# crockwell/rel_pose

Measured on AMD Instinct MI355X. Metric: image-pairs/sec fwd+bwd @384x384, 1/2/4/8 MI355X; R,t err vs ref, higher is better.
Workload: dtype f32; 1 GPU; train.py step (ViTEss fwd + geodesic loss + bwd + grad all-reduce + clip + Adam), synthetic 384x384 pairs; scope=full, pairs_per_gpu=64, global_batch_pairs=64, parallelism=dp1, finite=True, gemm_operand_precision=exact fp32 MFMA, launch=eager

## Files before the change

### rel_pose_amd/csrc/attention.hip

```cpp
#include "common.h"
#include "../../include/relpose_hip.h"
#include <stdlib.h>
#include <type_traits>

namespace {

template <int OFF> RP_DEV float lds_rd32(unsigned addr) {
  float v;
  asm volatile("ds_read_b32 %0, %1 offset:%2" : "=v"(v) : "v"(addr), "n"(OFF));
  return v;
}
template <int N, class F> RP_DEV void static_for(F&& f) {
  if constexpr (N > 0) {
    static_for<N - 1>(f);
    f(std::integral_constant<int, N - 1>{});
  }
}

constexpr int NTOK = 576;
constexpr int KST = 68;
constexpr int NTILE = NTOK / 32;

struct AttnP {
  const float* q; const float* k; const float* v;
  float* o; float* lse;
  int H, ldq, ldk, ldv, ldo, q_xor, k_xor;
  float scale;
  int ZH;
  float* colpart;
  float* pst;
  float* mrun;
};

template <int NT>
RP_DEV void tile_gload(const float* base, int ld, int tid, float4 (&r)[(512 + NT - 1) / NT]) {
#pragma unroll
  for (int j = 0; j < (512 + NT - 1) / NT; ++j) {
    int f = tid + NT * j;
    if (512 % NT != 0) f = min(f, 511);
    r[j] = ld4(base + (long long)(f >> 4) * ld + (f & 15) * 4);
  }
}
template <int NT, int STRIDE>
RP_DEV void tile_sstore(float* s, int tid, const float4 (&r)[(512 + NT - 1) / NT]) {
#pragma unroll
  for (int j = 0; j < (512 + NT - 1) / NT; ++j) {
    int f = tid + NT * j;
    if (512 % NT != 0) f = min(f, 511);
    st4(s + (f >> 4) * STRIDE + (f & 15) * 4, r[j]);
  }
}

template <bool BF>
RP_DEV f32x16 score_tile(const float* Ks, int l31, int hi, const float (&breg)[32], const bf16x8 (&bpk)[4]) {
  f32x16 s = zero16();
  const float* kr = Ks + l31 * KST + 32 * hi;
  if (BF) {
#pragma unroll
    for (int c = 0; c < 4; ++c) {
      const float4 x = ld4(kr + 8 * c), y = ld4(kr + 8 * c + 4);
      s = mfma_bf(pack8(x.x, x.y, x.z, x.w, y.x, y.y, y.z, y.w), bpk[c], s);
    }
    return s;
  }
#pragma unroll
  for (int c = 0; c < 8; ++c) {
    const float4 kf = ld4(kr + 4 * c);
    s = mfma32(kf.x, breg[4 * c + 0], s);
    s = mfma32(kf.y, breg[4 * c + 1], s);
    s = mfma32(kf.z, breg[4 * c + 2], s);
    s = mfma32(kf.w, breg[4 * c + 3], s);
  }
  return s;
}

template <int STRIDE, bool BF>
RP_DEV void accum_tile(const float* Ts, int l31, int hi, const f32x16& p, f32x16& o0, f32x16& o1) {
  if (BF) {
#pragma unroll
    for (int g = 0; g < 2; ++g) {
      float a0[8], a1[8];
#pragma unroll
      for (int j = 0; j < 8; ++j) {
        const float* vr = Ts + acc_row(8 * g + j, hi) * STRIDE + l31;
        a0[j] = vr[0];
        a1[j] = vr[32];
      }
      const bf16x8 pb = pack8(p[8 * g], p[8 * g + 1], p[8 * g + 2], p[8 * g + 3], p[8 * g + 4], p[8 * g + 5], p[8 * g + 6], p[8 * g + 7]);
      o0 = mfma_bf(pack8(a0), pb, o0);
      o1 = mfma_bf(pack8(a1), pb, o1);
    }
    return;
  }
#pragma unroll
  for (int r = 0; r < 16; ++r) {
    const float* vr = Ts + acc_row(r, hi) * STRIDE + l31;
    o0 = mfma32(vr[0], p[r], o0);
    o1 = mfma32(vr[32], p[r], o1);
  }
}

RP_DEV void store_ownerT(float* row_ptr, int hi, const f32x16& o0, const f32x16& o1, float mul) {
#pragma unroll
  for (int g = 0; g < 4; ++g) {
    st4(row_ptr + 8 * g + 4 * hi, make_float4(o0[4 * g] * mul, o0[4 * g + 1] * mul, o0[4 * g + 2] * mul, o0[4 * g + 3] * mul));
    st4(row_ptr + 32 + 8 * g + 4 * hi, make_float4(o1[4 * g] * mul, o1[4 * g + 1] * mul, o1[4 * g + 2] * mul, o1[4 * g + 3] * mul));
  }
}

RP_DEV void colsum_ownerT(float* part, int l31, int hi, const f32x16& o0, const f32x16& o1, float mul) {
#pragma unroll
  for (int r = 0; r < 16; ++r) {
    float a = row16_sum(o0[r]), b = row16_sum(o1[r]);
    a += __shfl_xor(a, 16, 64);
    b += __shfl_xor(b, 16, 64);
    if (l31 == 0) {
      part[acc_row(r, hi)] = a * mul;
      part[32 + acc_row(r, hi)] = b * mul;
    }
  }
}

RP_DEV void load_owner(const float* row_ptr, int hi, float mul, float (&reg)[32]) {
#pragma unroll
  for (int c = 0; c < 8; ++c) {
    const float4 x = ld4(row_ptr + 32 * hi + 4 * c);
    reg[4 * c + 0] = x.x * mul; reg[4 * c + 1] = x.y * mul; reg[4 * c + 2] = x.z * mul; reg[4 * c + 3] = x.w * mul;
  }
}

RP_DEV void pack_owner(const float (&reg)[32], bf16x8 (&pk)[4]) {
#pragma unroll
  for (int c = 0; c < 4; ++c) pk[c] = pack8(&reg[8 * c]);
}

template <bool NTS = true>
RP_DEV void store_tile_runs(float* tile, const f32x16& v, int lane) {
  typedef float f4v __attribute__((ext_vector_type(4)));
#pragma unroll
  for (int g = 0; g < 4; ++g) {
    const f4v x = {v[4 * g], v[4 * g + 1], v[4 * g + 2], v[4 * g + 3]};
    if (NTS) __builtin_nontemporal_store(x, reinterpret_cast<f4v*>(tile + 4 * (64 * g + lane)));
    else *reinterpret_cast<f4v*>(tile + 4 * (64 * g + lane)) = x;
  }
}

template <int NW, bool STATS, int WPS, bool BF, bool COLS = false, bool SAVEP = false>
__global__ __launch_bounds__(NW * 64, WPS) void attn_fwd_kernel(AttnP p) {
  constexpr int NT = NW * 64;
  constexpr int NPF = (512 + NT - 1) / NT;
  __shared__ __attribute__((aligned(16))) float Ks[2][32 * KST];
  __shared__ __attribute__((aligned(16))) float Vs[STATS ? 1 : 2][STATS ? 4 : 32 * 64];
  const int tid = threadIdx.x, lane = tid & 63, wave = tid >> 6, l31 = lane & 31, hi = lane >> 5;
  int zh, qblk;
  if (!xcd_problem(NTILE / NW, p.ZH, zh, qblk)) return;
  const int h = zh % p.H, z = zh / p.H;
  const int q0 = (qblk * NW + wave) * 32;
  const float* qb = p.q + (long long)(z ^ p.q_xor) * NTOK * p.ldq + h * 64;
  const float* kb = p.k + (long long)(z ^ (p.k_xor & 1)) * NTOK * p.ldk + h * 64;
  const float* vb = STATS ? nullptr : p.v + (long long)(z ^ (p.k_xor >> 1)) * NTOK * p.ldv + h * 64;

  float qreg[32];
  load_owner(qb + (long long)(q0 + l31) * p.ldq, hi, p.scale * RP_LOG2E, qreg);
  bf16x8 qpk[4];
  if (BF) pack_owner(qreg, qpk);

  f32x16 o0 = zero16(), o1 = zero16();
  float m = -INFINITY, l = 0.f;

  float4 kpre[NPF], vpre[NPF];
  tile_gload<NT>(kb, p.ldk, tid, kpre);
  if (!STATS) tile_gload<NT>(vb, p.ldv, tid, vpre);
  tile_sstore<NT, KST>(Ks[0], tid, kpre);
  if (!STATS) tile_sstore<NT, 64>(Vs[0], tid, vpre);
  __syncthreads();

  const int krow = l31 * KST + 32 * hi;
  float4 ka[4], kb2[4];
#pragma unroll
  for (int c = 0; c < 4; ++c) ka[c] = ld4(Ks[0] + krow + 4 * c);

  tile_gload<NT>(kb + (long long)32 * p.ldk, p.ldk, tid, kpre);
  if (!STATS) tile_gload<NT>(vb + (long long)32 * p.ldv, p.ldv, tid, vpre);

  for (int t = 0; t < NTILE; ++t) {
    const int cur = t & 1;
    const bool more = t + 1 < NTILE;
    float va[16], vb_[16];
#pragma unroll
    for (int c = 0; c < 4; ++c) kb2[c] = ld4(Ks[cur] + krow + 16 + 4 * c);
    if (!STATS) {
#pragma unroll
      for (int r = 0; r < 8; ++r) {
        const float* vr = Vs[cur] + acc_row(r, hi) * 64 + l31;
        va[2 * r] = vr[0];
        va[2 * r + 1] = vr[32];
      }
    }
    __builtin_amdgcn_sched_barrier(0);
    f32x16 s = zero16();
    if (BF) {
      s = mfma_bf(pack8(ka[0].x, ka[0].y, ka[0].z, ka[0].w, ka[1].x, ka[1].y, ka[1].z, ka[1].w), qpk[0], s);
      s = mfma_bf(pack8(ka[2].x, ka[2].y, ka[2].z, ka[2].w, ka[3].x, ka[3].y, ka[3].z, ka[3].w), qpk[1], s);
      s = mfma_bf(pack8(kb2[0].x, kb2[0].y, kb2[0].z, kb2[0].w, kb2[1].x, kb2[1].y, kb2[1].z, kb2[1].w), qpk[2], s);
      s = mfma_bf(pack8(kb2[2].x, kb2[2].y, kb2[2].z, kb2[2].w, kb2[3].x, kb2[3].y, kb2[3].z, kb2[3].w), qpk[3], s);
    } else {
#pragma unroll
    for (int c = 0; c < 4; ++c) {
      s = mfma32(ka[c].x, qreg[4 * c + 0], s);
      s = mfma32(ka[c].y, qreg[4 * c + 1], s);
      s = mfma32(ka[c].z, qreg[4 * c + 2], s);
      s = mfma32(ka[c].w, qreg[4 * c + 3], s);
    }
#pragma unroll
    for (int c = 0; c < 4; ++c) {
      s = mfma32(kb2[c].x, qreg[16 + 4 * c + 0], s);
      s = mfma32(kb2[c].y, qreg[16 + 4 * c + 1], s);
      s = mfma32(kb2[c].z, qreg[16 + 4 * c + 2], s);
      s = mfma32(kb2[c].w, qreg[16 + 4 * c + 3], s);
    }
    }
    if (STATS && SAVEP)
      store_tile_runs<false>(p.pst + (((long long)zh * NTILE + (q0 >> 5)) * NTILE + t) * 1024, s, lane);
    if (COLS) {
      float2* cp = reinterpret_cast<float2*>(p.colpart) + ((long long)zh * NTILE + (q0 >> 5)) * NTOK + t * 32;
#pragma unroll
      for (int r = 0; r < 16; ++r) {
        float cm = row16_max(s[r]);
        cm = fmaxf(cm, __shfl_xor(cm, 16, 64));
        float cl = row16_sum(fast_exp2(s[r] - cm));
        cl += __shfl_xor(cl, 16, 64);
        cp[acc_row(r, hi)] = make_float2(cm, cl);
      }
    }
    float mx = s[0];
#pragma unroll
    for (int r = 1; r < 16; ++r) mx = fmaxf(mx, s[r]);
    mx = fmaxf(mx, __shfl_xor(mx, 32, 64));
    const float mn = fmaxf(m, mx);
    const float alpha = fast_exp2(m - mn);
    m = mn;
    float ps = 0.f;
#pragma unroll
    for (int r = 0; r < 16; ++r) {
      s[r] = fast_exp2(s[r] - mn);
      ps += s[r];
    }
    l = l * alpha + ps;
    if (SAVEP && !STATS) {
      store_tile_runs(p.pst + (((long long)zh * NTILE + (q0 >> 5)) * NTILE + t) * 1024, s, lane);
      p.mrun[((long long)zh * NTILE + t) * NTOK + q0 + l31] = mn;
    }
    if (!STATS) {
#pragma unroll
      for (int r = 0; r < 8; ++r) {
        const float* vr = Vs[cur] + acc_row(8 + r, hi) * 64 + l31;
        vb_[2 * r] = vr[0];
        vb_[2 * r + 1] = vr[32];
      }
#pragma unroll
      for (int r = 0; r < 16; ++r) {
        o0[r] *= alpha;
        o1[r] *= alpha;
      }
      __builtin_amdgcn_sched_barrier(0);
      if (BF) {
        const bf16x8 pb = pack8(s[0], s[1], s[2], s[3], s[4], s[5], s[6], s[7]);
        o0 = mfma_bf(pack8(va[0], va[2], va[4], va[6], va[8], va[10], va[12], va[14]), pb, o0);
        o1 = mfma_bf(pack8(va[1], va[3], va[5], va[7], va[9], va[11], va[13], va[15]), pb, o1);
      } else {
#pragma unroll
      for (int r = 0; r < 8; ++r) {
        o0 = mfma32(va[2 * r], s[r], o0);
        o1 = mfma32(va[2 * r + 1], s[r], o1);
      }
      }
    }
    if (more) {
      tile_sstore<NT, KST>(Ks[cur ^ 1], tid, kpre);
      if (!STATS) tile_sstore<NT, 64>(Vs[cur ^ 1], tid, vpre);
    }
    __syncthreads();
    if (more) {
#pragma unroll
      for (int c = 0; c < 4; ++c) ka[c] = ld4(Ks[cur ^ 1] + krow + 4 * c);
      if (t + 2 < NTILE) {
        tile_gload<NT>(kb + (long long)(t + 2) * 32 * p.ldk, p.ldk, tid, kpre);
        if (!STATS) tile_gload<NT>(vb + (long long)(t + 2) * 32 * p.ldv, p.ldv, tid, vpre);
      }
    }
    if (!STATS) {
      __builtin_amdgcn_sched_barrier(0);
      if (BF) {
        const bf16x8 pb = pack8(s[8], s[9], s[10], s[11], s[12], s[13], s[14], s[15]);
        o0 = mfma_bf(pack8(vb_[0], vb_[2], vb_[4], vb_[6], vb_[8], vb_[10], vb_[12], vb_[14]), pb, o0);
        o1 = mfma_bf(pack8(vb_[1], vb_[3], vb_[5], vb_[7], vb_[9], vb_[11], vb_[13], vb_[15]), pb, o1);
      } else {
#pragma unroll
      for (int r = 0; r < 8; ++r) {
        o0 = mfma32(vb_[2 * r], s[8 + r], o0);
        o1 = mfma32(vb_[2 * r + 1], s[8 + r], o1);
      }
      }
    }
  }
  const float lt = l + __shfl_xor(l, 32, 64);
  if (!STATS) store_ownerT(p.o + ((long long)z * NTOK + q0 + l31) * p.ldo + h * 64, hi, o0, o1, 1.0f / lt);
  if (hi == 0) p.lse[((long long)z * p.H + h) * NTOK + q0 + l31] = m * RP_LN2 + logf(lt);
}

struct AttnBwdP {
  const float* q; const float* k; const float* v; const float* dout; const float* lse; const float* delta;
  float* dq; float* dk; float* dv;
  int H, ldq, ldk, ldv, lddo, lddq, lddk, lddv;
  float scale;
  int ZH;
  int kv_xor;
  float* ds;
  float *dk_colpart, *dv_colpart;
  int ldp;
  const float* pst;
  const float* mrun;
};

#ifdef RP_DKDV_PROBE
__device__ unsigned long long g_probe[16];
#define STAMP(i) { const unsigned long long now_ = __builtin_readcyclecounter(); acc_[i] += now_ - last_; last_ = now_; }
#else
#define STAMP(i)
#endif
template <int NW, int WPS, bool BF>
__global__ __launch_bounds__(NW * 64, WPS) void attn_bwd_dkdv_kernel(AttnBwdP p) {
#ifdef RP_DKDV_PROBE
  unsigned long long acc_[8] = {0, 0, 0, 0, 0, 0, 0, 0}, last_ = __builtin_readcyclecounter();
#endif
  constexpr int NT = NW * 64;
  constexpr int NPF = (512 + NT - 1) / NT;
  __shared__ __attribute__((aligned(16))) float Qs[2][32 * KST];
  __shared__ __attribute__((aligned(16))) float Ds[2][32 * KST];
  __shared__ __attribute__((aligned(16))) float Ls[2][64];
  __shared__ __attribute__((aligned(16))) float Tst[BF ? 1 : NW][BF ? 4 : 512];
  const int tid = threadIdx.x, lane = tid & 63, wave = tid >> 6, l31 = lane & 31, hi = lane >> 5;
  int zh, qblk;
  if (!xcd_problem(NTILE / NW, p.ZH, zh, qblk)) return;
  const int h = zh % p.H, z = zh / p.H;
  const int k0 = (qblk * NW + wave) * 32;
  const int zq = z ^ p.kv_xor;
  const float* qb = p.q + (long long)zq * NTOK * p.ldq + h * 64;
  const float* dob = p.dout + (long long)zq * NTOK * p.lddo + h * 64;
  const float* lseb = p.lse + ((long long)zq * p.H + h) * NTOK;
  const float* delb = p.delta + ((long long)zq * p.H + h) * NTOK;

  float kreg[32], vreg[32];
  load_owner(p.k + ((long long)z * NTOK + k0 + l31) * p.ldk + h * 64, hi, p.scale * RP_LOG2E, kreg);
  load_owner(p.v + ((long long)z * NTOK + k0 + l31) * p.ldv + h * 64, hi, 1.0f, vreg);
  bf16x8 kpk[4], vpk[4];
  if (BF) { pack_owner(kreg, kpk); pack_owner(vreg, vpk); }

  f32x16 dv0 = zero16(), dv1 = zero16(), dk0 = zero16(), dk1 = zero16();
  float4 qpre[NPF], dpre[NPF];
  float lpre = 0.f;
  tile_gload<NT>(qb, p.ldq, tid, qpre);
  tile_gload<NT>(dob, p.lddo, tid, dpre);
  const float* lsrc = (lane & 32) ? delb + (lane & 31) : lseb + (lane & 31);
  const float lmul = (lane & 32) ? 1.0f : RP_LOG2E;
  lpre = lsrc[0] * lmul;
  tile_sstore<NT, KST>(Qs[0], tid, qpre);
  tile_sstore<NT, KST>(Ds[0], tid, dpre);
  if (tid < 64) Ls[0][tid] = lpre;
  __syncthreads();

  STAMP(0)
  for (int t = 0; t < NTILE; ++t) {
    const int cur = t & 1;
    if (t + 1 < NTILE) {
      tile_gload<NT>(qb + (long long)(t + 1) * 32 * p.ldq, p.ldq, tid, qpre);
      tile_gload<NT>(dob + (long long)(t + 1) * 32 * p.lddo, p.lddo, tid, dpre);
      lpre = lsrc[(t + 1) * 32] * lmul;
    }
    STAMP(1)
    f32x16 s = score_tile<BF>(Qs[cur], l31, hi, kreg, kpk);
    f32x16 dp = score_tile<BF>(Ds[cur], l31, hi, vreg, vpk);
#ifdef RP_DKDV_PROBE
    asm volatile("" : "+v"(s), "+v"(dp));
#endif
    STAMP(2)
#pragma unroll
    for (int r = 0; r < 16; ++r) {
      const int qi = acc_row(r, hi);
      const float pr = fast_exp2(s[r] - Ls[cur][qi]);
      s[r] = pr;
      dp[r] = pr * (dp[r] - Ls[cur][32 + qi]);
    }
#ifdef RP_DKDV_PROBE
    asm volatile("" : "+v"(s), "+v"(dp));
#endif
    STAMP(3)
    if (p.ds) {
      const long long tile = (((long long)zq * p.H + h) * NTILE + t) * NTILE + (k0 >> 5);
      if (BF) store_acc_image_bf16(reinterpret_cast<unsigned short*>(p.ds) + tile * 1024, dp, p.scale, lane);
      else store_acc_image_lds(p.ds + tile * 1024, Tst[BF ? 0 : wave], dp, p.scale, lane);
    }
    STAMP(4)
    accum_tile<KST, BF>(Ds[cur], l31, hi, s, dv0, dv1);
    accum_tile<KST, BF>(Qs[cur], l31, hi, dp, dk0, dk1);
#ifdef RP_DKDV_PROBE
    asm volatile("" : "+v"(dv0), "+v"(dv1), "+v"(dk0), "+v"(dk1));
#endif
    STAMP(5)
    if (t + 1 < NTILE) {
      tile_sstore<NT, KST>(Qs[cur ^ 1], tid, qpre);
      tile_sstore<NT, KST>(Ds[cur ^ 1], tid, dpre);
      if (tid < 64) Ls[cur ^ 1][tid] = lpre;
    }
    STAMP(6)
    __syncthreads();
    STAMP(7)
  }
#ifdef RP_DKDV_PROBE
  if (lane == 0) { for (int i = 0; i < 8; ++i) atomicAdd(&g_probe[i], acc_[i]); atomicAdd(&g_probe[8], 1ull); }
#endif
  store_ownerT(p.dv + ((long long)z * NTOK + k0 + l31) * p.lddv + h * 64, hi, dv0, dv1, 1.0f);
  store_ownerT(p.dk + ((long long)z * NTOK + k0 + l31) * p.lddk + h * 64, hi, dk0, dk1, p.scale);
  if (p.dk_colpart) {
    const long long prow = ((long long)z * NTILE + (k0 >> 5)) * p.ldp + h * 64;
    colsum_ownerT(p.dv_colpart + prow, l31, hi, dv0, dv1, 1.0f);
    colsum_ownerT(p.dk_colpart + prow, l31, hi, dk0, dk1, p.scale);
  }
}

template <int NW, int WPS>
__global__ __launch_bounds__(NW * 64, WPS) void attn_bwd_dkdv_p_kernel(AttnBwdP p) {
#ifdef RP_DKDV_PROBE
  unsigned long long acc_[8] = {0, 0, 0, 0, 0, 0, 0, 0}, last_ = __builtin_readcyclecounter();
#endif
  constexpr int NT = NW * 64;
  constexpr int NPF = (512 + NT - 1) / NT;
  __shared__ __attribute__((aligned(16))) float Qs[2][32 * KST];
  __shared__ __attribute__((aligned(16))) float Ds[2][32 * KST];
  __shared__ __attribute__((aligned(16))) float Ls[2][NW][64];
  const int tid = threadIdx.x, lane = tid & 63, wave = tid >> 6, l31 = lane & 31, hi = lane >> 5;
  int zh, qblk;
  if (!xcd_problem(NTILE / NW, p.ZH, zh, qblk)) return;
  const int h = zh % p.H, z = zh / p.H;
  const int kb = qblk * NW + wave, k0 = kb * 32;
  const float* qb = p.q + (long long)z * NTOK * p.ldq + h * 64;
  const float* dob = p.dout + (long long)z * NTOK * p.lddo + h * 64;
  const float* lseb = p.lse + (long long)zh * NTOK;
  const float* delb = p.delta + (long long)zh * NTOK;
  const float* mb = p.mrun + ((long long)zh * NTILE + kb) * NTOK;
  const float* pt = p.pst + ((long long)zh * NTILE * NTILE + kb) * 1024 + (l31 >> 2) * 128 + (l31 & 3) + 16 * hi;
  float* dst = p.ds + ((long long)zh * NTILE * NTILE + kb) * 1024;

  float vreg[32];
  load_owner(p.v + ((long long)z * NTOK + k0 + l31) * p.ldv + h * 64, hi, p.scale, vreg);
  const bf16x8 nopk[4] = {};
  f32x16 dv0 = zero16(), dv1 = zero16(), dk0 = zero16(), dk1 = zero16();
  float4 qpre[NPF], dpre[NPF];
  const float* asrc = (lane & 32) ? delb + l31 : lseb + l31;
  const float* bsrc = (lane & 32) ? delb + l31 : mb + l31;
  const float km = (lane & 32) ? p.scale : 0.f, ke = (lane & 32) ? 0.f : 1.f;
  auto lfac = [&](float a, float b) { return fmaf(km, a, ke * fast_exp2(ke * fmaf(-a, RP_LOG2E, b))); };
  auto pload = [&](f32x16& x, int t) {
    const float* tp = pt + (long long)t * (NTILE * 1024);
#pragma unroll
    for (int r = 0; r < 16; ++r) x[r] = tp[acc_row(r, 0) * 4];
  };
  f32x16 pa, pb;
  tile_gload<NT>(qb, p.ldq, tid, qpre);
  tile_gload<NT>(dob, p.lddo, tid, dpre);
  float la = asrc[0], lb = bsrc[0];
  pload(pa, 0);
  tile_sstore<NT, KST>(Qs[0], tid, qpre);
  tile_sstore<NT, KST>(Ds[0], tid, dpre);
  Ls[0][wave][lane] = lfac(la, lb);
  __syncthreads();

  auto step = [&](f32x16& pc, f32x16& pn, int t) {
    const int cur = t & 1;
    if (t + 1 < NTILE) {
      tile_gload<NT>(qb + (long long)(t + 1) * 32 * p.ldq, p.ldq, tid, qpre);
      tile_gload<NT>(dob + (long long)(t + 1) * 32 * p.lddo, p.lddo, tid, dpre);
      la = asrc[(t + 1) * 32];
      lb = bsrc[(t + 1) * 32];
      pload(pn, t + 1);
    }
    STAMP(1)
    f32x16 dp = score_tile<false>(Ds[cur], l31, hi, vreg, nopk);
#ifdef RP_DKDV_PROBE
    asm volatile("" : "+v"(dp));
#endif
    STAMP(2)
    const float* L = Ls[cur][wave];
#pragma unroll
    for (int r = 0; r < 16; ++r) {
      const int qi = acc_row(r, hi);
      pc[r] *= L[qi];
      dp[r] = pc[r] * (dp[r] - L[32 + qi]);
    }
#ifdef RP_DKDV_PROBE
    asm volatile("" : "+v"(dp), "+v"(pc));
#endif
    STAMP(3)
    store_tile_runs(dst + (long long)t * (NTILE * 1024), dp, lane);
    STAMP(4)
    accum_tile<KST, false>(Ds[cur], l31, hi, pc, dv0, dv1);
    accum_tile<KST, false>(Qs[cur], l31, hi, dp, dk0, dk1);
#ifdef RP_DKDV_PROBE
    asm volatile("" : "+v"(dv0), "+v"(dv1), "+v"(dk0), "+v"(dk1));
#endif
    STAMP(5)
    if (t + 1 < NTILE) {
      tile_sstore<NT, KST>(Qs[cur ^ 1], tid, qpre);
      tile_sstore<NT, KST>(Ds[cur ^ 1], tid, dpre);
      Ls[cur ^ 1][wave][lane] = lfac(la, lb);
    }
    STAMP(6)
    __syncthreads();
    STAMP(7)
  };
  for (int t = 0; t < NTILE; t += 2) {
    step(pa, pb, t);
    step(pb, pa, t + 1);
  }
#ifdef RP_DKDV_PROBE
  if (lane == 0) { for (int i = 0; i < 8; ++i) atomicAdd(&g_probe[i], acc_[i]); atomicAdd(&g_probe[8], 1ull); }
#endif
  store_ownerT(p.dv + ((long long)z * NTOK + k0 + l31) * p.lddv + h * 64, hi, dv0, dv1, 1.0f);
  store_ownerT(p.dk + ((long long)z * NTOK + k0 + l31) * p.lddk + h * 64, hi, dk0, dk1, 1.0f);
  if (p.dk_colpart) {
    const long long prow = ((long long)z * NTILE + kb) * p.ldp + h * 64;
    colsum_ownerT(p.dv_colpart + prow, l31, hi, dv0, dv1, 1.0f);
    colsum_ownerT(p.dk_colpart + prow, l31, hi, dk0, dk1, 1.0f);
  }
}

template <int NW, int WPS, bool BF>
__global__ __launch_bounds__(NW * 64, WPS) void attn_bwd_dq_kernel(AttnBwdP p) {
  constexpr int NT = NW * 64;
  constexpr int NPF = (512 + NT - 1) / NT;
  __shared__ __attribute__((aligned(16))) float Ks[2][32 * KST];
  __shared__ __attribute__((aligned(16))) float Vs[2][32 * KST];
  const int tid = threadIdx.x, lane = tid & 63, wave = tid >> 6, l31 = lane & 31, hi = lane >> 5;
  int zh, qblk;
  if (!xcd_problem(NTILE / NW, p.ZH, zh, qblk)) return;
  const int h = zh % p.H, z = zh / p.H;
  const int q0 = (qblk * NW + wave) * 32;
  const float* kb = p.k + (long long)(z ^ p.kv_xor) * NTOK * p.ldk + h * 64;
  const float* vb = p.v + (long long)(z ^ p.kv_xor) * NTOK * p.ldv + h * 64;

  float qreg[32], dreg[32];
  load_owner(p.q + ((long long)z * NTOK + q0 + l31) * p.ldq + h * 64, hi, p.scale * RP_LOG2E, qreg);
  load_owner(p.dout + ((long long)z * NTOK + q0 + l31) * p.lddo + h * 64, hi, 1.0f, dreg);
  bf16x8 qpk[4], dpk[4];
  if (BF) { pack_owner(qreg, qpk); pack_owner(dreg, dpk); }
  const float lse = p.lse[((long long)z * p.H + h) * NTOK + q0 + l31] * RP_LOG2E;
  const float del = p.delta[((long long)z * p.H + h) * NTOK + q0 + l31];

  f32x16 dq0 = zero16(), dq1 = zero16();
  float4 kpre[NPF], vpre[NPF];
  tile_gload<NT>(kb, p.ldk, tid, kpre);
  tile_gload<NT>(vb, p.ldv, tid, vpre);
  tile_sstore<NT, KST>(Ks[0], tid, kpre);
  tile_sstore<NT, KST>(Vs[0], tid, vpre);
  __syncthreads();
  for (int t = 0; t < NTILE; ++t) {
    const int cur = t & 1;
    if (t + 1 < NTILE) {
      tile_gload<NT>(kb + (long long)(t + 1) * 32 * p.ldk, p.ldk, tid, kpre);
      tile_gload<NT>(vb + (long long)(t + 1) * 32 * p.ldv, p.ldv, tid, vpre);
    }
    f32x16 s = score_tile<BF>(Ks[cur], l31, hi, qreg, qpk);
    f32x16 dp = score_tile<BF>(Vs[cur], l31, hi, dreg, dpk);
#pragma unroll
    for (int r = 0; r < 16; ++r) dp[r] = fast_exp2(s[r] - lse) * (dp[r] - del);
    accum_tile<KST, BF>(Ks[cur], l31, hi, dp, dq0, dq1);
    if (t + 1 < NTILE) {
      tile_sstore<NT, KST>(Ks[cur ^ 1], tid, kpre);
      tile_sstore<NT, KST>(Vs[cur ^ 1], tid, vpre);
    }
    __syncthreads();
  }
  store_ownerT(p.dq + ((long long)z * NTOK + q0 + l31) * p.lddq + h * 64, hi, dq0, dq1, p.scale);
}

struct DsMmP {
  const float* ds; const float* b; float* out;
  int H, ldb, ldo, b_xor, ZH;
  int reverse;
  float* colpart;
  int ldp;
};

RP_DEV void accum_rows16(const float* Ts, int l31, int hi, const f32x16& p, f32x16& o0, f32x16& o1) {
#pragma unroll
  for (int r = 0; r < 16; ++r) {
    const float* vr = Ts + (16 * hi + r) * 64 + l31;
    o0 = mfma32(vr[0], p[r], o0);
    o1 = mfma32(vr[32], p[r], o1);
  }
}

template <int NW>
__global__ __launch_bounds__(NW * 64, 4) void ds_matmul_kernel(DsMmP p) {
  constexpr int NT = NW * 64;
  constexpr int KT = 32;
  constexpr int NSTEP = NTOK / KT;
  constexpr int NPF = (KT * 16 + NT - 1) / NT;
  __shared__ __attribute__((aligned(16))) float Bs[2][KT * 64];
  const int tid = threadIdx.x, lane = tid & 63, wave = tid >> 6, l31 = lane & 31, hi = lane >> 5;
  int zh, blk;
  if (!xcd_problem(NTILE / NW, p.ZH, zh, blk)) return;
  if (p.reverse) zh = p.ZH - 1 - zh;
  const int h = zh % p.H, z = zh / p.H;
  const int i0 = (blk * NW + wave) * 32;
  const float* bb = p.b + (long long)(z ^ p.b_xor) * NTOK * p.ldb + h * 64;
  const float* arow = p.ds + ((long long)zh * NTILE + (i0 >> 5)) * NTILE * 1024 + ((l31 & 3) + 4 * (l31 >> 3)) * 64 + 32 * ((l31 >> 2) & 1) + 16 * hi;

  f32x16 o0 = zero16(), o1 = zero16();
  float4 bpre[NPF];
  constexpr int NA = KT / 8;
  float4 a0[NA], a1[NA], a2[NA];
  auto aload = [&](float4 (&a)[NA], int t) {
#pragma unroll
    for (int g = 0; g < NA; ++g) {
      const float* src = arow + 1024 * ((KT / 32) * t + (g >> 2)) + 4 * (g & 3);
      a[g] = ld4(src);
    }
  };
  auto bload = [&](int t) {
#pragma unroll
    for (int j = 0; j < NPF; ++j) {
      int f = tid + NT * j;
      if ((KT * 16) % NT != 0) f = min(f, KT * 16 - 1);
      bpre[j] = ld4(bb + (long long)(t * KT + (f >> 4)) * p.ldb + (f & 15) * 4);
    }
  };
  auto bstore = [&](float* dst) {
#pragma unroll
    for (int j = 0; j < NPF; ++j) {
      int f = tid + NT * j;
      if ((KT * 16) % NT != 0) f = min(f, KT * 16 - 1);
      st4(dst + f * 4, bpre[j]);
    }
  };
  bload(0);
  aload(a0, 0);
  aload(a1, 1);
  bstore(Bs[0]);
  __syncthreads();
  bload(1);
  auto step = [&](const float4 (&a)[NA], float4 (&anext)[NA], int t) {
    const int cur = t & 1;
    if (t + 2 < NSTEP) aload(anext, t + 2);
#pragma unroll
    for (int u = 0; u < KT / 32; ++u) {
      f32x16 pr;
#pragma unroll
      for (int g = 0; g < 4; ++g) { pr[4 * g] = a[4 * u + g].x; pr[4 * g + 1] = a[4 * u + g].y; pr[4 * g + 2] = a[4 * u + g].z; pr[4 * g + 3] = a[4 * u + g].w; }
      accum_rows16(Bs[cur] + u * 32 * 64, l31, hi, pr, o0, o1);
    }
    if (t + 1 < NSTEP) bstore(Bs[cur ^ 1]);
    __syncthreads();
    if (t + 2 < NSTEP) bload(t + 2);
  };
  for (int t = 0; t < NSTEP; t += 3) {
    step(a0, a2, t);
    step(a1, a0, t + 1);
    step(a2, a1, t + 2);
  }
  store_ownerT(p.out + ((long long)z * NTOK + i0 + l31) * p.ldo + h * 64, hi, o0, o1, 1.0f);
  if (p.colpart) colsum_ownerT(p.colpart + ((long long)z * NTILE + (i0 >> 5)) * p.ldp + h * 64, l31, hi, o0, o1, 1.0f);
}

template <int NW>
__global__ __launch_bounds__(NW * 64, 3) void ds_matmul_t_kernel(DsMmP p) {
  __shared__ __attribute__((aligned(16))) float Bs[2][32 * 64];
  __shared__ __attribute__((aligned(16))) float Dt[NW][2][1024];
  const int tid = threadIdx.x, lane = tid & 63, wave = __builtin_amdgcn_readfirstlane(tid >> 6), l31 = lane & 31, hi = lane >> 5;
  int zh, blk;
  if (!xcd_problem(NTILE / NW, p.ZH, zh, blk)) return;
  if (p.reverse) zh = p.ZH - 1 - zh;
  const int h = zh % p.H, z = zh / p.H;
  const int ib = blk * NW + wave, i0 = ib * 32;
  const float* bb = p.b + (long long)(z ^ p.b_xor) * NTOK * p.ldb + h * 64;
  const float* tiles = p.ds + ((long long)zh * NTILE + ib) * NTILE * 1024;
  constexpr int BP = (8 + NW - 1) / NW;
  const unsigned dvoff = ((lane & 7) * 32 + (lane >> 3)) * 16, bvoff = (unsigned)((lane >> 4) * p.ldb * 4 + (lane & 15) * 16);
  const unsigned dt0 = lds_byte_addr(&Dt[wave][0][0]), bs0 = lds_byte_addr(&Bs[0][0]);
  auto issue = [&](int t, int buf) {
    const float* ts = tiles + (long long)t * 1024;
#pragma unroll
    for (int c = 0; c < 4; ++c) glds16(uniform_ptr(ts + 32 * c), dvoff, dt0 + buf * 4096 + c * 1024);
#pragma unroll
    for (int c = 0; c < BP; ++c) {
      const int piece = min(wave + NW * c, 7);
      glds16(uniform_ptr(bb + (long long)(t * 32 + 4 * piece) * p.ldb), bvoff, bs0 + buf * 8192 + piece * 1024);
    }
  };
  f32x16 o0 = zero16(), o1 = zero16();
  issue(0, 0);
  asm volatile("s_waitcnt vmcnt(0)" ::: "memory");
  __syncthreads();
  for (int t = 0; t < NTILE; ++t) {
    const int cur = t & 1;
    if (t + 1 < NTILE) issue(t + 1, cur ^ 1);
    const float* B = Bs[cur] + hi * 64 + l31;
    const float* D = Dt[wave][cur] + hi * 32 + l31;
#pragma unroll
    for (int s = 0; s < 16; ++s) {
      const float dsv = D[64 * s];
      o0 = mfma32(B[128 * s], dsv, o0);
      o1 = mfma32(B[128 * s + 32], dsv, o1);
    }
    asm volatile("s_waitcnt vmcnt(0)" ::: "memory");
    __syncthreads();
  }
  store_ownerT(p.out + ((long long)z * NTOK + i0 + l31) * p.ldo + h * 64, hi, o0, o1, 1.0f);
  if (p.colpart) colsum_ownerT(p.colpart + ((long long)z * NTILE + ib) * p.ldp + h * 64, l31, hi, o0, o1, 1.0f);
}

template <int NW>
__global__ __launch_bounds__(NW * 64, 3) void ds_matmul_t16_kernel(DsMmP p) {
  __shared__ __attribute__((aligned(16))) float Bs[2][32 * 64];
  __shared__ __attribute__((aligned(16))) float Dt[NW][2][1024];
  const int tid = threadIdx.x, lane = tid & 63, wave = __builtin_amdgcn_readfirstlane(tid >> 6), l15 = lane & 15, kq = lane >> 4;
  int zh, blk;
  if (!xcd_problem(NTILE / NW, p.ZH, zh, blk)) return;
  if (p.reverse) zh = p.ZH - 1 - zh;
  const int h = zh % p.H, z = zh / p.H;
  const int ib = blk * NW + wave, i0 = ib * 32;
  const float* bb = p.b + (long long)(z ^ p.b_xor) * NTOK * p.ldb + h * 64;
  const float* tiles = p.ds + ((long long)zh * NTILE + ib) * NTILE * 1024;
  constexpr int BP = (8 + NW - 1) / NW;
  const unsigned dvoff = ((((lane & 7) ^ (4 * ((lane >> 4) & 1))) * 32) + (lane >> 3)) * 16;
  const unsigned bvoff = (unsigned)((lane >> 4) * p.ldb * 4 + (((lane & 15) ^ (4 * (lane >> 4))) * 16));
  const unsigned dt0 = lds_byte_addr(&Dt[wave][0][0]), bs0 = lds_byte_addr(&Bs[0][0]);
  auto issue = [&](int t, int buf) {
    const float* ts = tiles + (long long)t * 1024;
#pragma unroll
    for (int c = 0; c < 4; ++c) glds16(uniform_ptr(ts + 32 * c), dvoff, dt0 + buf * 4096 + c * 1024);
#pragma unroll
    for (int c = 0; c < BP; ++c) {
      const int piece = min(wave + NW * c, 7);
      glds16(uniform_ptr(bb + (long long)(t * 32 + 4 * piece) * p.ldb), bvoff, bs0 + buf * 8192 + piece * 1024);
    }
  };
  f32x4 acc[4][2];
#pragma unroll
  for (int m = 0; m < 4; ++m)
#pragma unroll
    for (int n = 0; n < 2; ++n) acc[m][n] = f32x4{0.f, 0.f, 0.f, 0.f};
  int aoff[4], boff[2];
#pragma unroll
  for (int m = 0; m < 4; ++m) aoff[m] = kq * 64 + 16 * (m ^ kq) + l15;
#pragma unroll
  for (int n = 0; n < 2; ++n) boff[n] = kq * 32 + 16 * (n ^ (kq >> 1)) + l15;
  issue(0, 0);
  asm volatile("s_waitcnt vmcnt(0)" ::: "memory");
  __syncthreads();
  for (int t = 0; t < NTILE; ++t) {
    const int cur = t & 1;
    if (t + 1 < NTILE) issue(t + 1, cur ^ 1);
    const float* B = Bs[cur];
    const float* D = Dt[wave][cur];
#pragma unroll
    for (int ks = 0; ks < 8; ++ks) {
      float av[4], bv[2];
#pragma unroll
      for (int m = 0; m < 4; ++m) av[m] = B[ks * 256 + aoff[m]];
#pragma unroll
      for (int n = 0; n < 2; ++n) bv[n] = D[ks * 128 + boff[n]];
#pragma unroll
      for (int m = 0; m < 4; ++m)
#pragma unroll
        for (int n = 0; n < 2; ++n) acc[m][n] = __builtin_amdgcn_mfma_f32_16x16x4f32(av[m], bv[n], acc[m][n], 0, 0, 0);
    }
    asm volatile("s_waitcnt vmcnt(0)" ::: "memory");
    __syncthreads();
  }
#pragma unroll
  for (int n = 0; n < 2; ++n) {
    float* orow = p.out + ((long long)z * NTOK + i0 + 16 * n + l15) * p.ldo + h * 64 + 4 * kq;
#pragma unroll
    for (int m = 0; m < 4; ++m) st4(orow + 16 * m, make_float4(acc[m][n][0], acc[m][n][1], acc[m][n][2], acc[m][n][3]));
  }
  if (p.colpart) {
    float* part = p.colpart + ((long long)z * NTILE + ib) * p.ldp + h * 64;
#pragma unroll
    for (int m = 0; m < 4; ++m)
#pragma unroll
      for (int e = 0; e < 4; ++e) {
        const float v = row16_sum(acc[m][0][e] + acc[m][1][e]);
        if (l15 == 0) part[16 * m + 4 * kq + e] = v;
      }
  }
}

template <int NW>
__global__ __launch_bounds__(NW * 64, 4) void ds_matmul_bf16_kernel(DsMmP p) {
  constexpr int NT = NW * 64;
  constexpr int NPF = (512 + NT - 1) / NT;
  __shared__ __attribute__((aligned(16))) float Bs[2][32 * 64];
  const int tid = threadIdx.x, lane = tid & 63, wave = tid >> 6, l31 = lane & 31, hi = lane >> 5;
  int zh, blk;
  if (!xcd_problem(NTILE / NW, p.ZH, zh, blk)) return;
  if (p.reverse) zh = p.ZH - 1 - zh;
  const int h = zh % p.H, z = zh / p.H;
  const int i0 = (blk * NW + wave) * 32;
  const float* bb = p.b + (long long)(z ^ p.b_xor) * NTOK * p.ldb + h * 64;
  const unsigned short* arow = reinterpret_cast<const unsigned short*>(p.ds) + ((long long)zh * NTILE + (i0 >> 5)) * NTILE * 1024 +
                               ((l31 & 3) + 4 * (l31 >> 3)) * 64 + 32 * ((l31 >> 2) & 1) + 16 * hi;
  f32x16 o0 = zero16(), o1 = zero16();
  float4 bpre[NPF];
  uint4 a0[2], a1[2], a2[2];
  auto aload = [&](uint4 (&a)[2], int t) {
    a[0] = *reinterpret_cast<const uint4*>(arow + 1024 * t);
    a[1] = *reinterpret_cast<const uint4*>(arow + 1024 * t + 8);
  };
  auto bload = [&](int t) {
#pragma unroll
    for (int j = 0; j < NPF; ++j) {
      int f = tid + NT * j;
      if (512 % NT != 0) f = min(f, 511);
      bpre[j] = ld4(bb + (long long)(t * 32 + (f >> 4)) * p.ldb + (f & 15) * 4);
    }
// ... 321 lines not shown
```

Baseline: 1998 image-pairs/sec.

## Stream Q/dO tiles into swizzled LDS via direct global-to-LDS loads in dK/dV kernel

Reworks the attention backward dK/dV (P-stored) kernel so the Q and dO tiles go straight from global memory into XOR-swizzled LDS buffers through direct global-to-LDS loads. This replaces the old path of loading into registers and then storing to padded shared memory. New swizzle-aware score and accumulate helpers read those buffers, and the next tile's loads are issued between the two accumulate phases. Global accesses use address_space(1) pointers with uniform bases, and the wave index is made scalar. The aim is to cut register pressure and VALU/LDS store traffic and to overlap loads with MFMA work. The cost is hand-placed waitcnt and scheduling code that is fragile to get right.

```diff
diff --git a/rel_pose_amd/csrc/attention.hip b/rel_pose_amd/csrc/attention.hip
--- a/rel_pose_amd/csrc/attention.hip
+++ b/rel_pose_amd/csrc/attention.hip
@@ -134,14 +134,18 @@
   for (int c = 0; c < 4; ++c) pk[c] = pack8(&reg[8 * c]);
 }
 
-template <bool NTS = true>
-RP_DEV void store_tile_runs(float* tile, const f32x16& v, int lane) {
+template <bool NTS = true, class TP = float*, class LT = int>
+RP_DEV void store_tile_runs(TP tile, const f32x16& v, LT lane) {
   typedef float f4v __attribute__((ext_vector_type(4)));
+  typedef decltype(reinterpret_cast<f4v*>((float*)nullptr)) generic_t;
+  typedef __attribute__((address_space(1))) f4v* global_t;
+  typedef std::conditional_t<std::is_same<TP, float*>::value, generic_t, global_t> vp_t;
+  const TP mine = tile + 4 * lane;
 #pragma unroll
   for (int g = 0; g < 4; ++g) {
     const f4v x = {v[4 * g], v[4 * g + 1], v[4 * g + 2], v[4 * g + 3]};
-    if (NTS) __builtin_nontemporal_store(x, reinterpret_cast<f4v*>(tile + 4 * (64 * g + lane)));
-    else *reinterpret_cast<f4v*>(tile + 4 * (64 * g + lane)) = x;
+    if (NTS) __builtin_nontemporal_store(x, (vp_t)(mine + 256 * g));
+    else *(vp_t)(mine + 256 * g) = x;
   }
 }
 
@@ -429,17 +433,41 @@
   }
 }
 
+typedef const __attribute__((address_space(1))) float* rp_gcptr_t;
+typedef __attribute__((address_space(1))) float* rp_gptr_t;
+RP_DEV rp_gcptr_t uniform_gptr(const float* p) { return (rp_gcptr_t)(unsigned long long)uniform_ptr(p); }
+RP_DEV f32x16 score_tile_sw(const float* T, const int (&sc)[8], const float (&breg)[32]) {
+  f32x16 s = zero16();
+#pragma unroll
+  for (int c = 0; c < 8; ++c) {
+    const float4 kf = ld4(T + sc[c]);
+    s = mfma32(kf.x, breg[4 * c + 0], s);
+    s = mfma32(kf.y, breg[4 * c + 1], s);
+    s = mfma32(kf.z, breg[4 * c + 2], s);
+    s = mfma32(kf.w, breg[4 * c + 3], s);
+  }
+  return s;
+}
+template <bool VOL>
+RP_DEV void accum_tile_sw(const float* T, const int (&ar)[4], const f32x16& p, f32x16& o0, f32x16& o1) {
+#pragma unroll
+  for (int r = 0; r < 16; ++r) {
+    typedef std::conditional_t<VOL, const volatile __attribute__((address_space(3))) float*, const float*> rd_t;
+    const rd_t vr = (rd_t)T + ar[r & 3] + (r >> 2) * 512;
+    const int b = (r >> 2) & 1;
+    o0 = mfma32(vr[32 * b], p[r], o0);
+    o1 = mfma32(vr[32 * (1 - b)], p[r], o1);
+  }
+}
+
 template <int NW, int WPS>
 __global__ __launch_bounds__(NW * 64, WPS) void attn_bwd_dkdv_p_kernel(AttnBwdP p) {
 #ifdef RP_DKDV_PROBE
   unsigned long long acc_[8] = {0, 0, 0, 0, 0, 0, 0, 0}, last_ = __builtin_readcyclecounter();
 #endif
-  constexpr int NT = NW * 64;
-  constexpr int NPF = (512 + NT - 1) / NT;
-  __shared__ __attribute__((aligned(16))) float Qs[2][32 * KST];
-  __shared__ __attribute__((aligned(16))) float Ds[2][32 * KST];
+  __shared__ __attribute__((aligned(16))) float Ts[2][2][32 * 64];
   __shared__ __attribute__((aligned(16))) float Ls[2][NW][64];
-  const int tid = threadIdx.x, lane = tid & 63, wave = tid >> 6, l31 = lane & 31, hi = lane >> 5;
+  const int tid = threadIdx.x, lane = tid & 63, wave = __builtin_amdgcn_readfirstlane(tid >> 6), l31 = lane & 31, hi = lane >> 5;
   int zh, qblk;
   if (!xcd_problem(NTILE / NW, p.ZH, zh, qblk)) return;
   const int h = zh % p.H, z = zh / p.H;
@@ -449,44 +477,65 @@
   const float* lseb = p.lse + (long long)zh * NTOK;
   const float* delb = p.delta + (long long)zh * NTOK;
   const float* mb = p.mrun + ((long long)zh * NTILE + kb) * NTOK;
-  const float* pt = p.pst + ((long long)zh * NTILE * NTILE + kb) * 1024 + (l31 >> 2) * 128 + (l31 & 3) + 16 * hi;
+  const float* ptile = p.pst + ((long long)zh * NTILE * NTILE + kb) * 1024;
+  const unsigned poff = (l31 >> 2) * 128 + (l31 & 3) + 16 * hi;
   float* dst = p.ds + ((long long)zh * NTILE * NTILE + kb) * 1024;
 
   float vreg[32];
   load_owner(p.v + ((long long)z * NTOK + k0 + l31) * p.ldv + h * 64, hi, p.scale, vreg);
-  const bf16x8 nopk[4] = {};
   f32x16 dv0 = zero16(), dv1 = zero16(), dk0 = zero16(), dk1 = zero16();
-  float4 qpre[NPF], dpre[NPF];
-  const float* asrc = (lane & 32) ? delb + l31 : lseb + l31;
-  const float* bsrc = (lane & 32) ? delb + l31 : mb + l31;
+  constexpr int NV = 4 / NW, NI = 8 / NW;
+  unsigned qvoff[NV], dvoff[NV];
+#pragma unroll
+  for (int j = 0; j < NV; ++j) {
+    const unsigned x = (((lane & 15) ^ (lane >> 4) ^ (4 * (j * NW + wave))) & 15) * 16;
+    qvoff[j] = (unsigned)((lane >> 4) * p.ldq * 4) + x;
+    dvoff[j] = (unsigned)((lane >> 4) * p.lddo * 4) + x;
+  }
+  const unsigned ts0 = lds_byte_addr(&Ts[0][0][0]) + wave * 1024;
+  const long long qstep = (long long)(4 * NW) * p.ldq, dstep = (long long)(4 * NW) * p.lddo;
+  auto issue = [&](int t, int buf) {
+    const float* qs = uniform_ptr(qb + (long long)(t * 32 + 4 * wave) * p.ldq);
+    const float* dd = uniform_ptr(dob + (long long)(t * 32 + 4 * wave) * p.lddo);
+#pragma unroll
+    for (int i = 0; i < NI; ++i) glds16(qs + i * qstep, qvoff[i % NV], ts0 + buf * 16384 + i * (NW * 1024));
+#pragma unroll
+    for (int i = 0; i < NI; ++i) glds16(dd + i * dstep, dvoff[i % NV], ts0 + buf * 16384 + 8192 + i * (NW * 1024));
+  };
+  int sc[8], ar[4];
+#pragma unroll
+  for (int c = 0; c < 8; ++c) sc[c] = l31 * 64 + (((8 * hi + c) ^ (l31 & 15)) << 2);
+#pragma unroll
+  for (int j = 0; j < 4; ++j) ar[j] = (j + 4 * hi) * 64 + ((((l31 >> 2) ^ (j + 4 * hi)) << 2) | (l31 & 3));
   const float km = (lane & 32) ? p.scale : 0.f, ke = (lane & 32) ? 0.f : 1.f;
-  auto lfac = [&](float a, float b) { return fmaf(km, a, ke * fast_exp2(ke * fmaf(-a, RP_LOG2E, b))); };
+  auto lfac = [&](float lse, float del, float m) { return fmaf(km, del, ke * fast_exp2(ke * fmaf(-lse, RP_LOG2E, m))); };
+  float la, ld, lm;
+  auto lload = [&](int t) {
+    la = (uniform_gptr(lseb + t * 32) + (unsigned)l31)[0];
+    ld = (uniform_gptr(delb + t * 32) + (unsigned)l31)[0];
+    lm = (uniform_gptr(mb + t * 32) + (unsigned)l31)[0];
+  };
   auto pload = [&](f32x16& x, int t) {
-    const float* tp = pt + (long long)t * (NTILE * 1024);
+    const rp_gcptr_t tp = uniform_gptr(ptile + (long long)t * (NTILE * 1024)) + poff;
 #pragma unroll
     for (int r = 0; r < 16; ++r) x[r] = tp[acc_row(r, 0) * 4];
   };
   f32x16 pa, pb;
-  tile_gload<NT>(qb, p.ldq, tid, qpre);
-  tile_gload<NT>(dob, p.lddo, tid, dpre);
-  float la = asrc[0], lb = bsrc[0];
+  issue(0, 0);
+  lload(0);
   pload(pa, 0);
-  tile_sstore<NT, KST>(Qs[0], tid, qpre);
-  tile_sstore<NT, KST>(Ds[0], tid, dpre);
-  Ls[0][wave][lane] = lfac(la, lb);
+  asm volatile("s_waitcnt vmcnt(0)" ::: "memory");
+  Ls[0][wave][lane] = lfac(la, ld, lm);
   __syncthreads();
 
-  auto step = [&](f32x16& pc, f32x16& pn, int t) {
-    const int cur = t & 1;
-    if (t + 1 < NTILE) {
-      tile_gload<NT>(qb + (long long)(t + 1) * 32 * p.ldq, p.ldq, tid, qpre);
-      tile_gload<NT>(dob + (long long)(t + 1) * 32 * p.lddo, p.lddo, tid, dpre);
-      la = asrc[(t + 1) * 32];
-      lb = bsrc[(t + 1) * 32];
-      pload(pn, t + 1);
-    }
+  auto step = [&](f32x16& pc, f32x16& pn, int t, auto curc) {
+    constexpr int cur = decltype(curc)::value;
+    const int tn = cur ? min(t + 1, NTILE - 1) : t + 1;
+    lload(tn);
+    pload(pn, tn);
+    asm volatile("" ::: "memory");
     STAMP(1)
-    f32x16 dp = score_tile<false>(Ds[cur], l31, hi, vreg, nopk);
+    f32x16 dp = score_tile_sw(Ts[cur][1], sc, vreg);
 #ifdef RP_DKDV_PROBE
     asm volatile("" : "+v"(dp));
 #endif
@@ -502,26 +551,25 @@
     asm volatile("" : "+v"(dp), "+v"(pc));
 #endif
     STAMP(3)
-    store_tile_runs(dst + (long long)t * (NTILE * 1024), dp, lane);
+    store_tile_runs((rp_gptr_t)uniform_gptr(dst + (long long)t * (NTILE * 1024)), dp, (unsigned)lane);
     STAMP(4)
-    accum_tile<KST, false>(Ds[cur], l31, hi, pc, dv0, dv1);
-    accum_tile<KST, false>(Qs[cur], l31, hi, dp, dk0, dk1);
+    accum_tile_sw<NW == 1>(Ts[cur][1], ar, pc, dv0, dv1);
+    issue(tn, cur ^ 1);
+    accum_tile_sw<NW == 1>(Ts[cur][0], ar, dp, dk0, dk1);
 #ifdef RP_DKDV_PROBE
     asm volatile("" : "+v"(dv0), "+v"(dv1), "+v"(dk0), "+v"(dk1));
 #endif
     STAMP(5)
-    if (t + 1 < NTILE) {
-      tile_sstore<NT, KST>(Qs[cur ^ 1], tid, qpre);
-      tile_sstore<NT, KST>(Ds[cur ^ 1], tid, dpre);
-      Ls[cur ^ 1][wave][lane] = lfac(la, lb);
-    }
+    asm volatile("" : "+v"(la), "+v"(ld), "+v"(lm));
+    Ls[cur ^ 1][wave][lane] = lfac(la, ld, lm);
+    asm volatile("s_waitcnt vmcnt(0)" ::: "memory");
     STAMP(6)
     __syncthreads();
     STAMP(7)
   };
   for (int t = 0; t < NTILE; t += 2) {
-    step(pa, pb, t);
-    step(pb, pa, t + 1);
+    step(pa, pb, t, std::integral_constant<int, 0>{});
+    step(pb, pa, t + 1, std::integral_constant<int, 1>{});
   }
 #ifdef RP_DKDV_PROBE
   if (lane == 0) { for (int i = 0; i < 8; ++i) atomicAdd(&g_probe[i], acc_[i]); atomicAdd(&g_probe[8], 1ull); }
```

Result: no change. 2005 image-pairs/sec (median of 6 runs) (+0.4%).
